# ChunLI-666/PointCloudProcessor

Hardware: AMD Instinct MI355X
Metric: Mpoints×frames/sec colorized (higher is better)
Workload: dtype f32/f64

## Files before the change

pointcloudprocessor_amd/csrc/pcp_colour.hip:

```cpp
#include <algorithm>
#include <cfloat>
#include <cstdlib>

#include "pcp_device.hpp"
#include "pcp_hsv.hpp"
#include "pcp_scan.hpp"

namespace pcp {

constexpr int kBlock = 256;
constexpr uint32_t kFltMaxBits = 0x7f7fffffu;

template <bool kCommon>
__device__ __forceinline__ DevCamera common_camera(const DevCamera &in) {
  DevCamera c = in;
  if constexpr (kCommon) {
    c.cull_mode = PCP_CULL_ZBUFFER;
    c.enable_zbuf = 1;
    c.pretest = 1;
    c.ds_fast = 1;
  }
  return c;
}
inline bool is_common_camera(const DevCamera &c) {
// ... 96 lines not shown
  double r = __builtin_amdgcn_rcp(b);
  r = fma(fma(-b, r, 1.0), r, r);
  r = fma(fma(-b, r, 1.0), r, r);
  return r;
}
__device__ __forceinline__ Interval iv_pad(Interval a) {
  const double e = 1e-12 * (fabs(a.lo) + fabs(a.hi)) + 1e-300;
  return {a.lo - e, a.hi + e};
}

__device__ __forceinline__ int tile_classify(const DevCamera &c, const DevFrame &fr, float4 sph) {
  const double cx = sph.x, cy = sph.y, cz = sph.z;
  const float *m = fr.w2c;
  const double X = (m[0] * cx + m[1] * cy) + (m[2] * cz + m[3]);
  const double Y = (m[4] * cx + m[5] * cy) + (m[6] * cz + m[7]);
  const double Z = (m[8] * cx + m[9] * cy) + (m[10] * cz + m[11]);
  const double mag = fr.norm_bound * (fabs(cx) + fabs(cy) + fabs(cz) + 3.0 * sph.w) + fabs(static_cast<double>(m[3])) +
                     fabs(static_cast<double>(m[7])) + fabs(static_cast<double>(m[11])) + 1e-3;
  const double rho = fr.norm_bound * static_cast<double>(sph.w) * (1.0 + 1e-6) + 1e-6 * mag;
  if (!(rho >= 0.0) || !isfinite(X + Y + Z + rho)) return 0;
  if (Z + rho <= 0.0) return 1;
  if (Z - rho <= 0.0) return 0;
  const Interval zi{Z - rho, Z + rho};
  if (!(zi.lo >= 1e-290)) return 0;
  const Interval iz{iv_rcp_pos(zi.hi) * (1.0 - 1e-13), iv_rcp_pos(zi.lo) * (1.0 + 1e-13)};
  const Interval xn = iv_pad(iv_mul_by_pos(Interval{X - rho, X + rho}, iz));
  const Interval yn = iv_pad(iv_mul_by_pos(Interval{Y - rho, Y + rho}, iz));
  const Interval x2 = iv_sqr(xn), y2 = iv_sqr(yn);
  const Interval r2 = iv_add(x2, y2);
  const Interval r4 = iv_mul_pos(r2, r2);
  const Interval r6 = iv_mul_pos(r2, r4);
  Interval rc = iv_add(iv_add(iv_scale(c.k1, r2), iv_scale(c.k2, r4)), iv_scale(c.k3, r6));
  rc.lo += 1.0;
  rc.hi += 1.0;
  const Interval t1 = iv_scale(2.0, iv_mul(xn, yn));
  const Interval t2 = iv_add(r2, iv_scale(2.0, x2));
  const Interval t3 = iv_add(r2, iv_scale(2.0, y2));
  const Interval xd = iv_pad(iv_add(iv_add(iv_mul(rc, xn), iv_scale(c.p1, t1)), iv_scale(c.p2, t2)));
  const Interval yd = iv_pad(iv_add(iv_add(iv_mul(rc, yn), iv_scale(c.p1, t3)), iv_scale(c.p2, t1)));
  Interval u = iv_pad(iv_scale(c.fx, xd)), v = iv_pad(iv_scale(c.fy, yd));
  u.lo += c.cx; u.hi += c.cx;
  v.lo += c.cy; v.hi += c.cy;
  if (!isfinite(u.lo + u.hi + v.lo + v.hi)) return 0;
  if (u.hi < static_cast<double>(c.u_lo) || u.lo > static_cast<double>(c.u_hi) ||
      v.hi < static_cast<double>(c.v_lo) || v.lo > static_cast<double>(c.v_hi))
    return 1;
  return (u.lo > static_cast<double>(c.u_lo) + 1.0 && u.hi < static_cast<double>(c.u_hi) - 1.0 &&
          v.lo > static_cast<double>(c.v_lo) + 1.0 && v.hi < static_cast<double>(c.v_hi) - 1.0)
             ? 2
             : 0;
}

constexpr int kTileGroup = 16;

__global__ __launch_bounds__(kBlock) void k_group_mask_flat(const float4 *__restrict__ spheres, int64_t groups, DevCamera cam,
                                                            const DevFrame *__restrict__ frames, int32_t n_frames,
                                                            int32_t w0, int32_t w1, int32_t words,
                                                            uint32_t *__restrict__ group_mask,
                                                            uint32_t *__restrict__ group_inside, int32_t cull_enabled,
                                                            int32_t *__restrict__ zeroed, int32_t n_zeroed,
                                                            unsigned long long *__restrict__ far_maps, int64_t far_cells) {
  const int64_t idx = static_cast<int64_t>(blockIdx.x) * kBlock + threadIdx.x;
  if (idx < n_zeroed) zeroed[idx] = 0;
  for (int64_t c = idx; c < far_cells; c += static_cast<int64_t>(gridDim.x) * kBlock) far_maps[c] = 0x7f7f7f7f7f7f7f7full;
  const int32_t nw = w1 - w0;
  const int64_t gw = idx >> 5;
  const int64_t group = gw / nw;
  const bool live = group < groups;
  const int32_t w = w0 + static_cast<int32_t>(gw - group * nw);
  const int32_t f = (w << 5) + static_cast<int32_t>(idx & 31);
  int cls = 1;
  if (live && f < n_frames) cls = cull_enabled ? tile_classify(cam, frames[f], spheres[group]) : 0;
  const unsigned long long m = __ballot(cls != 1), in = __ballot(cls == 2);
  if (live && (idx & 31) == 0) {
    group_mask[group * words + w] = static_cast<uint32_t>((threadIdx.x & 32) ? (m >> 32) : m);
    group_inside[group * words + w] = static_cast<uint32_t>((threadIdx.x & 32) ? (in >> 32) : in);
  }
}

__global__ __launch_bounds__(kBlock) void k_tile_mask_dense(const float4 *__restrict__ spheres, int64_t tiles,
                                                            DevCamera cam, const DevFrame *__restrict__ frames,
                                                            int32_t n_frames, int32_t w0, int32_t w1, int32_t words,
                                                            const uint32_t *__restrict__ group_mask,
                                                            const uint32_t *__restrict__ group_inside,
                                                            uint32_t *__restrict__ tile_mask,
                                                            uint32_t *__restrict__ inside_mask, int32_t cull_enabled) {
  const int lane = threadIdx.x & 63;
  const int32_t nw = w1 - w0;
  const int64_t gw = static_cast<int64_t>(blockIdx.x) * (kBlock / 64) + (threadIdx.x >> 6);
  const int64_t group = gw / nw;
  if (group >= (tiles + kTileGroup - 1) / kTileGroup) return;
  const int32_t w = w0 + static_cast<int32_t>(gw - group * nw);
  const int t = lane & 15, slot = lane >> 4;
  const int64_t tile = group * kTileGroup + t;
  const bool have = tile < tiles;
  uint32_t todo = __builtin_amdgcn_readfirstlane(group_mask[group * words + w]);
  const int32_t nb = n_frames - (w << 5);
  if (nb < 32) todo &= nb <= 0 ? 0u : ((1u << nb) - 1u);
  const uint32_t whole = __builtin_amdgcn_readfirstlane(group_inside[group * words + w]) & todo;
  todo &= ~whole;
  uint32_t word = whole, inside = whole;
  if (todo) {
    const float4 sph = spheres[have ? tile : tiles - 1];
    while (todo) {
      int32_t bit[4];
#pragma unroll
      for (int k = 0; k < 4; ++k) {
        bit[k] = todo ? __builtin_ctz(todo) : -1;
        todo &= todo - (todo ? 1u : 0u);
      }
      const int32_t b = slot == 0 ? bit[0] : slot == 1 ? bit[1] : slot == 2 ? bit[2] : bit[3];
      int cls = 1;
      if (b >= 0 && have) cls = cull_enabled ? tile_classify(cam, frames[(w << 5) + b], sph) : 0;
      const unsigned long long keep = __ballot(cls != 1), ins = __ballot(cls == 2);
#pragma unroll
      for (int k = 0; k < 4; ++k) {
        if (bit[k] >= 0) {
          word |= static_cast<uint32_t>((keep >> (k * 16 + t)) & 1ull) << bit[k];
          inside |= static_cast<uint32_t>((ins >> (k * 16 + t)) & 1ull) << bit[k];
        }
      }
    }
  }
  if (slot == 0 && have) {
    tile_mask[tile * words + w] = word;
    if (inside_mask) inside_mask[tile * words + w] = inside;
  }
}

constexpr int kWorkBins = 1024;
constexpr int kWorkPerBlock = 1024;
__global__ __launch_bounds__(kBlock) void k_tile_work_hist(const uint32_t *__restrict__ tile_mask, int64_t tiles, int32_t w0,
                                                          int32_t w1, int32_t words, int32_t *__restrict__ tile_work,
                                                          int32_t *__restrict__ hist) {
  __shared__ int32_t cnt[kWorkBins];
  for (int b = threadIdx.x; b < kWorkBins; b += kBlock) cnt[b] = 0;
  __syncthreads();
  const int64_t base = static_cast<int64_t>(blockIdx.x) * kWorkPerBlock;
  for (int q = 0; q < kWorkPerBlock / kBlock; ++q) {
    const int64_t t = base + q * kBlock + threadIdx.x;
    if (t < tiles) {
      int32_t visits = 0;
      for (int32_t w = w0; w < w1; ++w) visits += __builtin_popcount(tile_mask[t * words + w]);
      tile_work[t] = visits;
      atomicAdd(&cnt[min(visits, kWorkBins - 1)], 1);
    }
  }
  __syncthreads();
  for (int b = threadIdx.x; b < kWorkBins; b += kBlock)
    if (cnt[b]) atomicAdd(&hist[b], cnt[b]);
}
__device__ __forceinline__ int32_t block_exclusive_scan(int32_t v, int32_t *total);
__global__ __launch_bounds__(kBlock) void k_work_scatter(const int32_t *__restrict__ work, int64_t tiles,
                                                        const int32_t *__restrict__ hist, int32_t *__restrict__ cursor,
                                                        int32_t *__restrict__ order) {
  __shared__ int32_t cnt[kWorkBins];
  __shared__ int32_t first[kWorkBins];
  for (int b = threadIdx.x; b < kWorkBins; b += kBlock) cnt[b] = 0;
  {
    constexpr int kPer = kWorkBins / kBlock;
    int32_t h[kPer], mine = 0;
#pragma unroll
    for (int k = 0; k < kPer; ++k) {
      h[k] = hist[kWorkBins - 1 - (static_cast<int>(threadIdx.x) * kPer + k)];
      mine += h[k];
    }
    int32_t total = 0;
    int32_t run = block_exclusive_scan(mine, &total);
#pragma unroll
    for (int k = 0; k < kPer; ++k) {
      first[kWorkBins - 1 - (static_cast<int>(threadIdx.x) * kPer + k)] = run;
      run += h[k];
    }
  }
  __syncthreads();
  const int64_t base = static_cast<int64_t>(blockIdx.x) * kWorkPerBlock;
  int32_t bin[kWorkPerBlock / kBlock], rank[kWorkPerBlock / kBlock];
#pragma unroll
  for (int q = 0; q < kWorkPerBlock / kBlock; ++q) {
    const int64_t t = base + q * kBlock + threadIdx.x;
    bin[q] = t < tiles ? min(work[t], kWorkBins - 1) : -1;
    rank[q] = bin[q] >= 0 ? atomicAdd(&cnt[bin[q]], 1) : 0;
  }
  __syncthreads();
  for (int b = threadIdx.x; b < kWorkBins; b += kBlock)
    if (cnt[b]) cnt[b] = first[b] + atomicAdd(&cursor[b], cnt[b]);
  __syncthreads();
#pragma unroll
  for (int q = 0; q < kWorkPerBlock / kBlock; ++q)
    if (bin[q] >= 0) order[cnt[bin[q]] + rank[q]] = static_cast<int32_t>(base + q * kBlock + threadIdx.x);
}

constexpr uint32_t kXcdChunk = 16;
__device__ __forceinline__ uint32_t xcd_chunked_block() {
  constexpr uint32_t kXcd = 8, kSuper = kXcd * kXcdChunk;
  const uint32_t b = blockIdx.x;
  if (b >= (gridDim.x / kSuper) * kSuper) return b;
  const uint32_t x = b % kXcd, slot = b / kXcd;
  return ((slot / kXcdChunk) * kXcd + x) * kXcdChunk + slot % kXcdChunk;
}

constexpr unsigned long long kDepthEmpty = 0x7f7f7f7f7f7f7f7full;
__device__ __forceinline__ void depth_min(unsigned long long *__restrict__ map, int32_t cell, unsigned long long bits) {
  if (bits < map[cell]) atomicMin(map + cell, bits);
// ... 624 lines not shown
  if (need_frames && ctx->n_frames <= 0) return set_error(ctx, PCP_ERR_STATE, "%s: pcp_set_frames has not been called", who);
  hipError_t e = hipSetDevice(ctx->device);
  if (e != hipSuccess) return set_error(ctx, PCP_ERR_DEVICE, "%s: hipSetDevice failed: %s", who, hipGetErrorString(e));
  return PCP_OK;
}

static int check_frame(pcp_context *ctx, const char *who, int32_t frame) {
  if (frame < 0 || frame >= ctx->n_frames)
    return set_error(ctx, PCP_ERR_RANGE, "%s: keyframe %d out of range (0..%d)", who, frame, ctx->n_frames - 1);
  return PCP_OK;
}

static int fill_u32(pcp_context *ctx, uint32_t *p, int64_t n, uint32_t v) {
  if (n <= 0) return PCP_OK;
  LaunchTimer t(ctx, PCP_K_MISC);
  const uint32_t grid = static_cast<uint32_t>(std::min<int64_t>(div_up(n, kBlock), 8192));
  hipLaunchKernelGGL(k_fill_u32, dim3(grid), dim3(kBlock), 0, ctx->stream, p, n, v);
  PCP_HIP_TRY(ctx, hipGetLastError());
  return PCP_OK;
}

static int ensure_images(pcp_context *ctx) {
  const size_t px = static_cast<size_t>(ctx->dcam.img_w) * ctx->dcam.img_h;
  const size_t need = px * static_cast<size_t>(ctx->n_frames) + 4;
  if (ctx->images.count < need) {
    PCP_HIP_TRY(ctx, ctx->images.ensure(need));
    PCP_HIP_TRY(ctx, hipMemsetAsync(ctx->images.p, 0, need * 4, ctx->stream));
    ctx->image_set.assign(static_cast<size_t>(ctx->n_frames), 0);
    ctx->mask_set.assign(static_cast<size_t>(ctx->n_frames), 0);
  }
  return PCP_OK;
}

int wait_images(pcp_context *ctx, int32_t f0, int32_t f1) {
  ctx->texels_touched = true;
  if (ctx->image_pending.empty()) return PCP_OK;
  for (int lane = 0; lane < pcp_context::kUploadLanes; ++lane) {
    int32_t last = -1;
    for (int32_t f = std::max(f0, 0); f < f1 && f < static_cast<int32_t>(ctx->image_pending.size()); ++f) {
      const size_t sf = static_cast<size_t>(f);
      if (ctx->image_pending[sf] && ctx->image_lane[sf] == lane &&
          (last < 0 || ctx->image_seq[sf] > ctx->image_seq[static_cast<size_t>(last)]))
        last = f;
    }
    if (last < 0) continue;
    PCP_HIP_TRY(ctx, hipStreamWaitEvent(ctx->stream, ctx->image_event[static_cast<size_t>(last)], 0));
    const uint64_t seq = ctx->image_seq[static_cast<size_t>(last)];
    for (size_t f = 0; f < ctx->image_pending.size(); ++f)
      if (ctx->image_pending[f] && ctx->image_lane[f] == lane && ctx->image_seq[f] <= seq) ctx->image_pending[f] = 0;
  }
  return PCP_OK;
}

static int sort_tiles_by_work(pcp_context *ctx, int32_t w0, int32_t w1, int32_t *order) {
  const uint32_t sort_blocks = static_cast<uint32_t>(div_up(ctx->n_tiles, static_cast<int64_t>(kWorkPerBlock)));
  hipLaunchKernelGGL(k_tile_work_hist, dim3(sort_blocks), dim3(kBlock), 0, ctx->stream, ctx->tile_mask.p, ctx->n_tiles, w0, w1,
                     ctx->mask_words, ctx->tile_work.p, ctx->work_hist.p);
  hipLaunchKernelGGL(k_work_scatter, dim3(sort_blocks), dim3(kBlock), 0, ctx->stream, ctx->tile_work.p, ctx->n_tiles,
                     ctx->work_hist.p, ctx->work_hist.p + kWorkBins, order);
  PCP_HIP_TRY(ctx, hipGetLastError());
  return PCP_OK;
}

static int ensure_hull_bits(pcp_context *ctx) {
  const size_t words = static_cast<size_t>((ctx->n_frames + 31) / 32);
  const size_t need = words * static_cast<size_t>(ctx->n) + 4;
  if (ctx->hull_bits.count < need || ctx->hull_valid.size() != static_cast<size_t>(ctx->n_frames)) {
    PCP_HIP_TRY(ctx, ctx->hull_bits.ensure(need));
    ctx->hull_valid.assign(static_cast<size_t>(ctx->n_frames), 0);
  }
  return PCP_OK;
}

static int ensure_depth(pcp_context *ctx) {
  const size_t need = static_cast<size_t>(cells_of(ctx)) * ctx->n_frames + 4;
  if (ctx->depth.count < need) {
    PCP_HIP_TRY(ctx, ctx->depth.ensure(need));
    std::fill(ctx->depth_valid.begin(), ctx->depth_valid.end(), uint8_t(0));
  }
  const int32_t words = (ctx->n_frames + 31) / 32;
  const size_t need_mask = static_cast<size_t>(words) * static_cast<size_t>(std::max<int64_t>(ctx->n_tiles, 1)) + 4;
  if (ctx->tile_mask.count < need_mask || ctx->mask_words != words) {
    PCP_HIP_TRY(ctx, ctx->tile_mask.ensure(need_mask));
    PCP_HIP_TRY(ctx, ctx->tile_inside.ensure(need_mask));
    PCP_HIP_TRY(ctx, ctx->tile_work.ensure(static_cast<size_t>(std::max<int64_t>(ctx->n_tiles, 1)) + 4));
    PCP_HIP_TRY(ctx, ctx->tile_order.ensure(static_cast<size_t>(std::max<int64_t>(ctx->n_tiles, 1)) + 4));
    PCP_HIP_TRY(ctx, ctx->work_hist.ensure(2 * kWorkBins + 4));
    ctx->tile_order_live = false;
    ctx->mask_words = words;
    std::fill(ctx->depth_valid.begin(), ctx->depth_valid.end(), uint8_t(0));
  }
  return PCP_OK;
}

static int ensure_state(pcp_context *ctx) {
  const size_t sn = static_cast<size_t>(ctx->n);
  PCP_HIP_TRY(ctx, ctx->top_score.ensure(kTopM * sn + 4));
  PCP_HIP_TRY(ctx, ctx->top_rgb.ensure(kTopM * sn + 4));
  PCP_HIP_TRY(ctx, ctx->top_frame.ensure(kTopM * sn + 4));
  PCP_HIP_TRY(ctx, ctx->view_count.ensure(sn + 4));
  PCP_HIP_TRY(ctx, ctx->rgba2[0].ensure(sn + 4));
  PCP_HIP_TRY(ctx, ctx->rgba2[1].ensure(sn + 4));
  return PCP_OK;
}

int compact_flags(pcp_context *ctx, const uint8_t *flags, int64_t n, int32_t *out_index, int64_t capacity,
                  int64_t *count) {
  const int64_t tiles = std::max<int64_t>(1, div_up(n, kTile));
  PCP_HIP_TRY(ctx, ctx->s_tiles.ensure(static_cast<size_t>(tiles) + 4));
  PCP_HIP_TRY(ctx, ctx->s_counter.ensure(4));
  {
    LaunchTimer t(ctx, PCP_K_MISC);
    hipLaunchKernelGGL(k_tile_count, dim3(static_cast<uint32_t>(tiles)), dim3(kBlock), 0, ctx->stream, flags, n,
                       ctx->s_tiles.p);
    hipLaunchKernelGGL(k_scan_tiles, dim3(1), dim3(kScanTilesBlock), 0, ctx->stream, ctx->s_tiles.p, tiles, ctx->s_counter.p);
    if (out_index)
      hipLaunchKernelGGL(k_tile_scatter, dim3(static_cast<uint32_t>(tiles)), dim3(kBlock), 0, ctx->stream, flags, n,
                         ctx->s_tiles.p, out_index, capacity);
    PCP_HIP_TRY(ctx, hipGetLastError());
  }
  unsigned long long total = 0;
  unsigned long long *dst = ctx->readback ? static_cast<unsigned long long *>(ctx->readback) : &total;
  PCP_HIP_TRY(ctx, hipMemcpyAsync(dst, ctx->s_counter.p, sizeof(total), hipMemcpyDeviceToHost, ctx->stream));
  PCP_HIP_TRY(ctx, hipStreamSynchronize(ctx->stream));
  *count = static_cast<int64_t>(*dst);
  return PCP_OK;
}

static int single_frame_depth(pcp_context *ctx, int32_t frame) {
  const int64_t cells = cells_of(ctx);
  PCP_HIP_TRY(ctx, ctx->s_u32.ensure(static_cast<size_t>(cells) + 4));
  if (ctx->depth_from_batch) {
    if (!ctx->depth.p || static_cast<size_t>(frame) >= ctx->depth_valid.size() || !ctx->depth_valid[static_cast<size_t>(frame)])
      return set_error(ctx, PCP_ERR_STATE, "PCP_DEPTH_BATCHED: pcp_depth_pass has not covered keyframe %d", frame);
    PCP_HIP_TRY(ctx, hipMemcpyAsync(ctx->s_u32.p, ctx->depth.p + static_cast<int64_t>(frame) * cells,
                                    static_cast<size_t>(cells) * 4, hipMemcpyDeviceToDevice, ctx->stream));
    return PCP_OK;
  }
  if (ctx->n > 0 && ctx->dcam.enable_zbuf) {
    const size_t plane = plane_of(ctx);
// ... 465 lines not shown
    hipLaunchKernelGGL(k_gather_visible, dim3(blocks_for(take)), dim3(kBlock), 0, ctx->stream, ctx->xyz.p,
                       ctx->xyz.p + plane, ctx->xyz.p + 2 * plane, ctx->dcam, ctx->hframes[static_cast<size_t>(frame)],
                       ctx->s_cell.p, take, ctx->images.p + static_cast<int64_t>(frame) * px,
                       static_cast<int32_t>(ctx->image_set[static_cast<size_t>(frame)]),
                       static_cast<int32_t>(ctx->mask_set[static_cast<size_t>(frame)]),
                       reinterpret_cast<uint32_t *>(ctx->s_range.p), d_cam, d_world);
    PCP_HIP_TRY(ctx, hipGetLastError());
  }
  std::vector<uint32_t> rgbm;
  if (out_rgb || out_mask) {
    rgbm.resize(st);
    PCP_HIP_TRY(ctx, hipMemcpyAsync(rgbm.data(), ctx->s_range.p, st * 4, hipMemcpyDeviceToHost, ctx->stream));
  }
  if (out_index) PCP_HIP_TRY(ctx, hipMemcpyAsync(out_index, ctx->s_cell.p, st * 4, hipMemcpyDeviceToHost, ctx->stream));
  if (want_cam) PCP_HIP_TRY(ctx, hipMemcpyAsync(out_xyz_cam, d_cam, 3 * st * 4, hipMemcpyDeviceToHost, ctx->stream));
  if (want_world) PCP_HIP_TRY(ctx, hipMemcpyAsync(out_xyz_world, d_world, 3 * st * 4, hipMemcpyDeviceToHost, ctx->stream));
  PCP_HIP_TRY(ctx, hipStreamSynchronize(ctx->stream));
  for (size_t k = 0; k < rgbm.size(); ++k) {
    if (out_rgb) {
      out_rgb[3 * k + 0] = static_cast<uint8_t>(rgbm[k] & 0xffu);
      out_rgb[3 * k + 1] = static_cast<uint8_t>((rgbm[k] >> 8) & 0xffu);
      out_rgb[3 * k + 2] = static_cast<uint8_t>((rgbm[k] >> 16) & 0xffu);
    }
    if (out_mask) out_mask[k] = static_cast<uint16_t>(rgbm[k] >> 24);
  }
  return PCP_OK;
}

int pcp_depth_pass(pcp_context *ctx, int32_t frame_begin, int32_t frame_end) {
  int rc = check_ready(ctx, "pcp_depth_pass", true);
  if (rc != PCP_OK) return rc;
  if (frame_begin < 0 || frame_end > ctx->n_frames || frame_begin > frame_end)
    return set_error(ctx, PCP_ERR_RANGE, "pcp_depth_pass: keyframe range [%d,%d) outside 0..%d", frame_begin, frame_end,
                     ctx->n_frames);
  if (frame_begin == frame_end) return PCP_OK;
  if ((rc = ensure_depth(ctx)) != PCP_OK) return rc;
  const int64_t cells = cells_of(ctx);
  const int64_t map_cells = static_cast<int64_t>(frame_end - frame_begin) * cells;
  const bool z_maps = ctx->n > 0 && ctx->dcam.enable_zbuf;
  if (z_maps) {
    PCP_HIP_TRY(ctx, ctx->depth_sq.ensure(static_cast<size_t>(map_cells) + 4));
  } else if ((rc = fill_u32(ctx, ctx->depth.p + static_cast<int64_t>(frame_begin) * cells, map_cells, kFltMaxBits)) != PCP_OK) {
    return rc;
  }
  if (ctx->n > 0) {
    const size_t plane = plane_of(ctx);
    const int32_t w0 = frame_begin >> 5, w1 = ((frame_end - 1) >> 5) + 1;
    static const bool cull_tiles = [] {
      const char *e = std::getenv("PCP_DISABLE_TILE_CULL");
      return !(e && e[0] == '1');
    }();
    {
      LaunchTimer t(ctx, PCP_K_TILE_MASK);
      const int64_t groups = div_up(ctx->n_tiles, kTileGroup);
      const float4 *tile_sph = reinterpret_cast<const float4 *>(ctx->tile_sphere.p);
      const size_t gwords = static_cast<size_t>(groups) * ctx->mask_words;
      PCP_HIP_TRY(ctx, ctx->group_mask.ensure(2 * gwords + 8));
      uint32_t *group_inside = ctx->group_mask.p + gwords + 4;
      hipLaunchKernelGGL(k_group_mask_flat, dim3(std::max(blocks_for(groups * (w1 - w0) * 32), blocks_for(2 * kWorkBins))),
                         dim3(kBlock), 0, ctx->stream, tile_sph + ctx->n_tiles, groups, ctx->dcam, ctx->frames.p, ctx->n_frames,
                         w0, w1, ctx->mask_words, ctx->group_mask.p, group_inside, cull_tiles ? 1 : 0, ctx->work_hist.p,
                         2 * kWorkBins, z_maps ? reinterpret_cast<unsigned long long *>(ctx->depth_sq.p) : nullptr,
                         z_maps ? map_cells : int64_t(0));
      hipLaunchKernelGGL(k_tile_mask_dense, dim3(static_cast<uint32_t>(div_up(groups * (w1 - w0), kBlock / 64))), dim3(kBlock),
                         0, ctx->stream, tile_sph, ctx->n_tiles, ctx->dcam, ctx->frames.p, ctx->n_frames, w0, w1,
                         ctx->mask_words, ctx->group_mask.p, group_inside, ctx->tile_mask.p, ctx->tile_inside.p, cull_tiles ? 1 : 0);
      if ((rc = sort_tiles_by_work(ctx, w0, w1, ctx->tile_order.p)) != PCP_OK) return rc;
      ctx->tile_order_live = true;
    }
    if (ctx->cull.cull_mode == PCP_CULL_HPR) {
      int rch = ensure_hull_bits(ctx);
      if (rch != PCP_OK) return rch;
      if (!ctx->depth_from_batch) {
        int32_t clear_until = frame_begin;
        for (int32_t f = frame_begin; f < frame_end; ++f) {
          uint32_t *hull_plane = ctx->hull_bits.p + static_cast<size_t>(f >> 5) * static_cast<size_t>(ctx->n);
          if ((f & 31) == 0 && std::min(f + 32, ctx->n_frames) <= frame_end) {
            PCP_HIP_TRY(ctx, hipMemsetAsync(hull_plane, 0, static_cast<size_t>(ctx->n) * 4, ctx->stream));
            clear_until = std::min(f + 32, ctx->n_frames);
          }
          if (f >= clear_until) {
            LaunchTimer t(ctx, PCP_K_HPR);
            hipLaunchKernelGGL(k_hull_clear, dim3(blocks_for(ctx->n)), dim3(kBlock), 0, ctx->stream, hull_plane, ctx->n, 1u << (f & 31));
          }
        }
        PCP_HIP_TRY(ctx, hipGetLastError());
        const char *le = std::getenv("PCP_HPR_LANES");
        const int32_t lanes = le && le[0] >= '1' && le[0] <= '8' ? le[0] - '0' : 4;
        if ((rc = hpr_run_range(ctx, frame_begin, frame_end, lanes, ctx->tile_mask.p)) != PCP_OK) return rc;
        for (int32_t f = frame_begin; f < frame_end; ++f) ctx->hull_valid[static_cast<size_t>(f)] = 1;
      }
    }
    {
      LaunchTimer t(ctx, PCP_K_DEPTH);
      hipLaunchKernelGGL(is_common_camera(ctx->dcam) ? k_depth_pass<true> : k_depth_pass<false>,
                         dim3(static_cast<uint32_t>(ctx->n_tiles)), dim3(64), 0, ctx->stream, ctx->sxyz.p,
                         ctx->sxyz.p + plane, ctx->sxyz.p + 2 * plane, ctx->n, ctx->dcam, ctx->frames.p, frame_begin,
                         frame_end, ctx->depth_sq.p, cells, frame_begin, ctx->tile_mask.p, ctx->tile_inside.p,
                         ctx->mask_words, ctx->tile_order.p);
      if (z_maps)
        hipLaunchKernelGGL(k_depth_finish, dim3(static_cast<uint32_t>(std::min<int64_t>(div_up(map_cells, kBlock), 4096))),
                           dim3(kBlock), 0, ctx->stream, ctx->depth_sq.p, map_cells,
                           ctx->depth.p + static_cast<int64_t>(frame_begin) * cells);
      PCP_HIP_TRY(ctx, hipGetLastError());
    }
  }
  for (int32_t f = frame_begin; f < frame_end; ++f) ctx->depth_valid[static_cast<size_t>(f)] = 1;
  return PCP_OK;
}

int pcp_depth_maps_device(pcp_context *ctx, void **device_ptr, int64_t *n_floats) {
  int rc = check_ready(ctx, "pcp_depth_maps_device", true);
  if (rc != PCP_OK) return rc;
  if (ctx->cull.cull_mode == PCP_CULL_HPR)
    return set_error(ctx, PCP_ERR_STATE, "pcp_depth_maps_device: PCP_CULL_HPR has no depth maps to merge across point shards "
                     "(the hull needs the whole map on one GPU)");
  if ((rc = ensure_depth(ctx)) != PCP_OK) return rc;
  if (device_ptr) *device_ptr = ctx->depth.p;
  if (n_floats) *n_floats = cells_of(ctx) * ctx->n_frames;
  return PCP_OK;
// ... 427 lines not shown
```

pointcloudprocessor_amd/csrc/pcp_context.hip:

```cpp
#include <algorithm>
#include <cfloat>
#include <cmath>
#include <cstdlib>
#include <new>
#include <vector>

#include "pcp_internal.hpp"
#include "pcp_scan.hpp"

namespace pcp {

static thread_local std::string g_error;

int set_error(const pcp_context *ctx, int code, const char *fmt, ...) {
  char buf[1024];
  va_list ap;
  va_start(ap, fmt);
  vsnprintf(buf, sizeof(buf), fmt, ap);
  va_end(ap);
  if (ctx)
    ctx->error = buf;
  else
    g_error = buf;
  return code;
// ... 428 lines not shown

static int store_cloud(pcp_context *ctx, const float *x, const float *y, const float *z, int64_t n,
                       const void *aos = nullptr, int64_t stride = 0) {
  PCP_HIP_TRY(ctx, hipSetDevice(ctx->device));
  const size_t sn = static_cast<size_t>(n);
  const size_t plane = (sn + 3) & ~size_t(3);
  PCP_HIP_TRY(ctx, ctx->xyz.ensure(3 * plane + 4));
  PCP_HIP_TRY(ctx, ctx->sxyz.ensure(3 * plane + 4));
  PCP_HIP_TRY(ctx, ctx->perm.ensure(sn + 4));
  ctx->n = n;
  ctx->nonfinite_points = 0;
  ctx->sor_distances_live = false;
  ctx->sor_partial_slab = ctx->sor_partial_slabs = -1;
  ctx->n_tiles = 0;
  ctx->tile_order_live = false;
  ctx->have_intensity = false;
  ctx->nid_chunks = 0;
  ctx->colour_state_live = false;
  ctx->colour_result_live = false;
  ctx->labels_live = false;
  match_table_release(ctx);
  ctx->mls_count = 0;
  ctx->vgd_next = ctx->css_next = -1;
  ctx->css_ball = 0.0;
  std::fill(ctx->depth_valid.begin(), ctx->depth_valid.end(), uint8_t(0));
  ctx->hull_valid.clear();
  for (int a = 0; a < 3; ++a) ctx->host_min[a] = ctx->host_max[a] = 0.0f;
  if (n == 0) return PCP_OK;
  hipStream_t st = ctx->stream;
  float *dx = ctx->xyz.p, *dy = ctx->xyz.p + plane, *dz = ctx->xyz.p + 2 * plane;
  PCP_HIP_TRY(ctx, hipMemsetAsync(ctx->sxyz.p, 0, (3 * plane + 4) * 4, st));
  DevBuf<uint32_t> raw;
  if (aos) {
    PCP_HIP_TRY(ctx, raw.ensure(static_cast<size_t>(n) * static_cast<size_t>(stride) / 4 + 4));
    PCP_HIP_TRY(ctx, hipMemcpyAsync(raw.p, aos, static_cast<size_t>(n) * static_cast<size_t>(stride), hipMemcpyHostToDevice, st));
    hipLaunchKernelGGL(k_up_deinterleave, dim3(up_blocks(n)), dim3(kUpBlock), 0, st, raw.p, stride / 4, n, dx, dy, dz);
  } else {
    PCP_HIP_TRY(ctx, hipMemcpyAsync(dx, x, sn * 4, hipMemcpyHostToDevice, st));
    PCP_HIP_TRY(ctx, hipMemcpyAsync(dy, y, sn * 4, hipMemcpyHostToDevice, st));
    PCP_HIP_TRY(ctx, hipMemcpyAsync(dz, z, sn * 4, hipMemcpyHostToDevice, st));
  }
  float mn[3], mx[3];
  unsigned long long nonfinite = 0;
  PCP_HIP_TRY(ctx, ctx->inv_perm.ensure(plane + 4));
  if (int rc = spatial_order(ctx, dx, dy, dz, n, ctx->perm.p, ctx->sxyz.p, ctx->sxyz.p + plane, ctx->sxyz.p + 2 * plane,
                             ctx->inv_perm.p, mn, mx, &nonfinite))
    return rc;
  raw.release();
  ctx->nonfinite_points = static_cast<int64_t>(nonfinite);
  for (int a = 0; a < 3; ++a) {
    ctx->host_min[a] = mn[a];
    ctx->host_max[a] = mx[a];
  }
  const int64_t tiles = (n + 63) / 64, groups = (tiles + 15) / 16;
  PCP_HIP_TRY(ctx, ctx->tile_sphere.ensure(static_cast<size_t>(tiles + groups) * 4 + 4));
  float4 *sph = reinterpret_cast<float4 *>(ctx->tile_sphere.p);
  hipLaunchKernelGGL(k_up_spheres<64>, dim3(static_cast<uint32_t>((tiles + 3) / 4)), dim3(kUpBlock), 0, st, ctx->sxyz.p,
                     ctx->sxyz.p + plane, ctx->sxyz.p + 2 * plane, n, sph, tiles);
  hipLaunchKernelGGL(k_up_spheres<1024>, dim3(static_cast<uint32_t>(groups)), dim3(kUpBlock), 0, st, ctx->sxyz.p,
                     ctx->sxyz.p + plane, ctx->sxyz.p + 2 * plane, n, sph + tiles, groups);
  PCP_HIP_TRY(ctx, hipGetLastError());
  ctx->n_tiles = tiles;
  PCP_HIP_TRY(ctx, hipStreamSynchronize(st));
  return PCP_OK;
}

}

using namespace pcp;

extern "C" {

int pcp_abi_version(void) { return PCP_ABI_VERSION; }

int pcp_create(int32_t device, pcp_context **out) {
  if (!out) {
    set_global_error("pcp_create: out is NULL");
    return PCP_ERR_INVALID;
  }
  *out = nullptr;
  int count = 0;
  hipError_t e = hipGetDeviceCount(&count);
  if (e != hipSuccess || count <= 0) {
    set_global_error("pcp_create: no HIP device available (%s); libpcp_hip has no CPU fallback",
                     e == hipSuccess ? "device count 0" : hipGetErrorString(e));
    return PCP_ERR_DEVICE;
  }
  if (device < 0 || device >= count) {
    set_global_error("pcp_create: device %d out of range (0..%d)", device, count - 1);
    return PCP_ERR_INVALID;
  }
  e = hipSetDevice(device);
  if (e == hipSuccess) {
    hipFuncAttributes a;
    const hipError_t pl[] = {hipFuncGetAttributes(&a, reinterpret_cast<const void *>(&k_up_bbox)), preload_colour(), preload_mls(),
                             preload_nid(), preload_hpr(), preload_colour_smooth(), preload_match(),
                             preload_jpeg()};
    for (hipError_t x : pl)
      if (x != hipSuccess && e == hipSuccess) e = x;
  }
  if (e != hipSuccess) {
    set_global_error("pcp_create: hipSetDevice(%d) / loading the gfx950 code objects failed: %s", device, hipGetErrorString(e));
    return PCP_ERR_DEVICE;
  }
  pcp_context *ctx = new (std::nothrow) pcp_context();
  if (!ctx) {
    set_global_error("pcp_create: out of host memory");
    return PCP_ERR_NOMEM;
  }
  ctx->device = device;
  e = hipStreamCreateWithFlags(&ctx->own_stream, hipStreamNonBlocking);
  if (e != hipSuccess) {
    set_global_error("pcp_create: hipStreamCreate failed: %s", hipGetErrorString(e));
// ... 7 lines not shown
    if (e == hipSuccess) e = hipStreamCreateWithPriority(&ctx->copy_stream, hipStreamNonBlocking, prio_greatest);
  }
  for (int k = 0; k < 2 && e == hipSuccess; ++k) {
    e = hipEventCreateWithFlags(&ctx->result_ready[k], hipEventDisableTiming);
    if (e == hipSuccess) e = hipEventCreateWithFlags(&ctx->copy_done[k], hipEventDisableTiming);
  }
  if (e != hipSuccess) {
    set_global_error("pcp_create: copy stream / events: %s", hipGetErrorString(e));
    pcp_destroy(ctx);
    return PCP_ERR_DEVICE;
  }
  if (hipHostMalloc(&ctx->readback, pcp_context::kReadbackBytes, hipHostMallocDefault) != hipSuccess) {
    ctx->readback = nullptr;
    (void)hipGetLastError();
  }
  pcp_default_camera(&ctx->camera);
  pcp_default_cull_params(&ctx->cull);
  *out = ctx;
  return PCP_OK;
}

void pcp_destroy(pcp_context *ctx) {
  if (!ctx) return;
  (void)hipSetDevice(ctx->device);
  (void)hipStreamSynchronize(ctx->stream);
  if (ctx->copy_stream) (void)hipStreamSynchronize(ctx->copy_stream);
  for (hipStream_t us : ctx->upload_stream)
    if (us) {
      (void)hipStreamSynchronize(us);
      (void)hipStreamDestroy(us);
    }
  for (auto e : ctx->image_event)
    if (e) (void)hipEventDestroy(e);
  if (ctx->texels_idle) (void)hipEventDestroy(ctx->texels_idle);
  for (auto &b : ctx->upload_stage) b.release();
  for (auto &b : ctx->jpeg_planes) b.release();
  drain_timing(ctx);
  for (auto e : ctx->event_pool) (void)hipEventDestroy(e);
  ctx->xyz.release();
  ctx->sxyz.release();
  ctx->perm.release();
  ctx->inv_perm.release();
  ctx->frames.release();
  ctx->images.release();
  ctx->hsv_tables.release();
  ctx->depth.release();
  ctx->depth_sq.release();
  ctx->tile_sphere.release();
  ctx->tile_mask.release();
  ctx->tile_inside.release();
  ctx->tile_work.release();
  ctx->tile_order.release();
  ctx->work_hist.release();
  ctx->group_mask.release();
  ctx->top_score.release();
  ctx->top_rgb.release();
  ctx->top_frame.release();
  ctx->view_count.release();
  ctx->rgba2[0].release();
  ctx->rgba2[1].release();
  ctx->labels.release();
  match_table_release(ctx);
  ctx->match_moved.release();
  for (int k = 0; k < 2; ++k) {
    if (ctx->result_ready[k]) (void)hipEventDestroy(ctx->result_ready[k]);
    if (ctx->copy_done[k]) (void)hipEventDestroy(ctx->copy_done[k]);
  }
  if (ctx->copy_stream) (void)hipStreamDestroy(ctx->copy_stream);
  ctx->s_cell.release();
  ctx->s_pixel.release();
  ctx->s_range.release();
  ctx->s_cam.release();
  ctx->s_keep.release();
  ctx->s_u32.release();
  ctx->s_counter.release();
  ctx->s_tiles.release();
  ctx->g_cell.release();
  ctx->g_rank.release();
  ctx->g_start.release();
  ctx->g_occ.release();
  ctx->g_occ_rank.release();
  ctx->g_order.release();
  ctx->g_xyz.release();
  ctx->m_tmp.release();
  ctx->s_dist.release();
  ctx->css_dist.release();
  ctx->s_kth.release();
  ctx->css_words.release();
  ctx->m_state.release();
  ctx->slp_table.release();
  ctx->c_perm.release();
  ctx->m_flag.release();
  ctx->intensity.release();
  for (auto &lane : ctx->hpr_lane) lane.release();
  if (ctx->hpr_fork) (void)hipEventDestroy(ctx->hpr_fork);
  for (auto &e : ctx->hpr_join)
    if (e) (void)hipEventDestroy(e);
  ctx->hull_bits.release();
  ctx->nid_pts.release();
  ctx->nid_chunk_kf.release();
  ctx->nid_hist.release();
  ctx->m_sums.release();
  ctx->c_index.release();
  ctx->c_xyz.release();
  ctx->c_mark.release();
  ctx->c_where.release();
  ctx->c_xyz2.release();
// ... 299 lines not shown
```

pointcloudprocessor_amd/csrc/pcp_internal.hpp:

```cpp
#pragma once

#include <hip/hip_runtime.h>

#include <cstdarg>
#include <cstdint>
#include <chrono>
#include <cstdio>
#include <cstring>
#include <string>
#include <vector>

#include "pcp_hip.h"

namespace pcp {

struct DevCamera {
  double fx, fy, cx, cy;
  double k1, k2, p1, p2, k3;
  double slack;
  float ds_f;
  double img_wd, img_hd;
  float cull_wf, cull_hf;
  float ds_rcp;
  int32_t ds_fast;
// ... 107 lines not shown
}

struct pcp_context {
  int32_t device = 0;
  hipStream_t own_stream = nullptr;
  hipStream_t stream = nullptr;
  void *readback = nullptr;
  static constexpr size_t kReadbackBytes = 65536;
  mutable std::string error;

  bool have_camera = false;
  pcp_camera camera{};
  pcp_cull_params cull{};
  pcp::DevCamera dcam{};

  int64_t n = 0;
  int64_t nonfinite_points = 0;
  pcp::DevBuf<float> xyz;
  pcp::DevBuf<float> sxyz;
  pcp::DevBuf<int32_t> perm;
  pcp::DevBuf<int32_t> inv_perm;
  std::vector<float> host_min = {0, 0, 0}, host_max = {0, 0, 0};

  int32_t n_frames = 0;
  std::vector<pcp_pose> poses;
  std::vector<pcp::DevFrame> hframes;
  pcp::DevBuf<pcp::DevFrame> frames;
  pcp::DevBuf<uint32_t> images;
  std::vector<uint8_t> image_set, mask_set;
  static constexpr int kUploadLanes = 2;
  hipStream_t upload_stream[kUploadLanes] = {nullptr, nullptr};
  pcp::DevBuf<uint8_t> upload_stage[kUploadLanes];
  pcp::DevBuf<uint8_t> jpeg_planes[kUploadLanes];
  std::vector<hipEvent_t> image_event;
  std::vector<uint8_t> image_pending;
  std::vector<uint8_t> image_lane;
  std::vector<uint64_t> image_seq;
  bool lane_must_wait[kUploadLanes] = {false, false};
  uint64_t upload_seq = 0;
  uint64_t upload_turn = 0;
  hipEvent_t texels_idle = nullptr;
  bool texels_touched = false;
  bool adjust_images = false;
  float saturation_scale = 1.0f, brightness_scale = 1.0f;
  pcp::DevBuf<int32_t> hsv_tables;

  pcp::DevBuf<uint32_t> depth;
  pcp::DevBuf<unsigned long long> depth_sq;
  std::vector<uint8_t> depth_valid;
  bool depth_from_batch = false;

  int64_t n_tiles = 0;
  pcp::DevBuf<float> tile_sphere;
  pcp::DevBuf<uint32_t> tile_mask, group_mask;
  pcp::DevBuf<uint32_t> tile_inside;
  int32_t mask_words = 0;
  pcp::DevBuf<int32_t> tile_work, tile_order, work_hist;
  bool tile_order_live = false;

  pcp::DevBuf<float> top_score;
  pcp::DevBuf<uint32_t> top_rgb;
  pcp::DevBuf<int32_t> top_frame;
  pcp::DevBuf<int32_t> view_count;
  pcp::DevBuf<uint32_t> rgba2[2];
  int32_t rgba_cur = 0;
  hipStream_t copy_stream = nullptr;
  hipEvent_t result_ready[2] = {nullptr, nullptr}, copy_done[2] = {nullptr, nullptr};
  bool copy_pending[2] = {false, false};
  bool colour_state_live = false;
  bool colour_result_live = false;
  bool label_fusion = false;
  bool labels_live = false;
  pcp::DevBuf<uint32_t> labels;

  bool match_live = false;
  double match_e = 0.0, match_rc = 0.0;
  float match_e2 = 0.0f;
  int64_t match_a = 0;
  int64_t match_entries = 0;
  pcp::DevBuf<uint8_t> match_in_a;
  pcp::DevBuf<int32_t> match_list;
  pcp::DevBuf<int64_t> match_off;
  pcp::DevBuf<int32_t> match_cols;
  pcp::DevBuf<unsigned long long> match_moved;

  pcp::DevBuf<int32_t> s_cell, s_pixel;
  pcp::DevBuf<float> s_range, s_cam;
  pcp::DevBuf<uint8_t> s_keep;
  pcp::DevBuf<uint32_t> s_u32;
  pcp::DevBuf<unsigned long long> s_counter;
  pcp::DevBuf<int32_t> s_tiles;

  static constexpr int kHprMaxLanes = 8;
  pcp::HprLane hpr_lane[kHprMaxLanes];
  int32_t hpr_last_lane = 0;
  hipEvent_t hpr_fork = nullptr, hpr_join[kHprMaxLanes] = {};
  pcp::DevBuf<uint32_t> hull_bits;
  std::vector<uint8_t> hull_valid;
  int64_t hpr_stats[10] = {0, 0, 0, 0, 0, 0, 0, 0, 0, 0};
  bool hpr_stats_pending = false;

  pcp::DevBuf<int32_t> g_cell, g_rank, g_start, g_order;
  pcp::DevBuf<unsigned long long> g_occ;
  pcp::DevBuf<int32_t> g_occ_rank;
  pcp::DevBuf<float> g_xyz;
  pcp::DevBuf<float> m_tmp;
  pcp::DevBuf<float> s_dist;
  pcp::DevBuf<double> m_state;
  double slp_radius = 0.05, slp_step = 0.01;
  pcp::DevBuf<float> slp_table;
// ... 145 lines not shown
```

Before: 1.871 million.

## Fuse hierarchical tile culling, work histogram into one three-level mask kernel

Replaces the separate group-mask, dense tile-mask and work-histogram kernels with one kernel per block of tile groups. It adds a third, coarser level of bounding spheres (16 groups each) and culls hierarchically with shared-memory append lists. The histogram is computed in the same kernel, and its counters are double-buffered so each launch zeroes the next set. This removes two launches and a global re-read of the tile masks, and skips per-tile tests for frames rejected at the upper or group level. The cost is heavier shared-memory use and serialized loops over frame chunks within each block.

New measurement: 1.901 million, median of 6. Within noise of the previous version (+1.6%).

```diff
diff --git a/pointcloudprocessor_amd/csrc/pcp_colour.hip b/pointcloudprocessor_amd/csrc/pcp_colour.hip
--- a/pointcloudprocessor_amd/csrc/pcp_colour.hip
+++ b/pointcloudprocessor_amd/csrc/pcp_colour.hip
@@ -172,104 +172,127 @@
 }
 
 constexpr int kTileGroup = 16;
-
-__global__ __launch_bounds__(kBlock) void k_group_mask_flat(const float4 *__restrict__ spheres, int64_t groups, DevCamera cam,
-                                                            const DevFrame *__restrict__ frames, int32_t n_frames,
-                                                            int32_t w0, int32_t w1, int32_t words,
-                                                            uint32_t *__restrict__ group_mask,
-                                                            uint32_t *__restrict__ group_inside, int32_t cull_enabled,
-                                                            int32_t *__restrict__ zeroed, int32_t n_zeroed,
-                                                            unsigned long long *__restrict__ far_maps, int64_t far_cells) {
-  const int64_t idx = static_cast<int64_t>(blockIdx.x) * kBlock + threadIdx.x;
-  if (idx < n_zeroed) zeroed[idx] = 0;
-  for (int64_t c = idx; c < far_cells; c += static_cast<int64_t>(gridDim.x) * kBlock) far_maps[c] = 0x7f7f7f7f7f7f7f7full;
-  const int32_t nw = w1 - w0;
-  const int64_t gw = idx >> 5;
-  const int64_t group = gw / nw;
-  const bool live = group < groups;
-  const int32_t w = w0 + static_cast<int32_t>(gw - group * nw);
-  const int32_t f = (w << 5) + static_cast<int32_t>(idx & 31);
-  int cls = 1;
-  if (live && f < n_frames) cls = cull_enabled ? tile_classify(cam, frames[f], spheres[group]) : 0;
-  const unsigned long long m = __ballot(cls != 1), in = __ballot(cls == 2);
-  if (live && (idx & 31) == 0) {
-    group_mask[group * words + w] = static_cast<uint32_t>((threadIdx.x & 32) ? (m >> 32) : m);
-    group_inside[group * words + w] = static_cast<uint32_t>((threadIdx.x & 32) ? (in >> 32) : in);
-  }
-}
-
-__global__ __launch_bounds__(kBlock) void k_tile_mask_dense(const float4 *__restrict__ spheres, int64_t tiles,
-                                                            DevCamera cam, const DevFrame *__restrict__ frames,
-                                                            int32_t n_frames, int32_t w0, int32_t w1, int32_t words,
-                                                            const uint32_t *__restrict__ group_mask,
-                                                            const uint32_t *__restrict__ group_inside,
-                                                            uint32_t *__restrict__ tile_mask,
-                                                            uint32_t *__restrict__ inside_mask, int32_t cull_enabled) {
+constexpr int kUpperGroups = 16;
+#ifndef PCP_MASK_GROUPS
+#define PCP_MASK_GROUPS 4
+#endif
+constexpr int kMaskGroups = PCP_MASK_GROUPS;
+constexpr int kMaskTiles = kMaskGroups * kTileGroup;
+constexpr int kMaskChunkWords = kBlock / 32;
+static_assert(kUpperGroups % kMaskGroups == 0 && kMaskTiles <= kBlock, "a workgroup lies within one upper group");
+#ifndef PCP_MASK_UPPER
+#define PCP_MASK_UPPER 1
+#endif
+constexpr bool kMaskUpper = PCP_MASK_UPPER != 0;
+constexpr int kWorkBins = 1024;
+
+__device__ __forceinline__ void wave_append(bool take, uint16_t v, uint16_t *list, int32_t *count) {
+  const unsigned long long b = __ballot(take);
+  if (!b) return;
   const int lane = threadIdx.x & 63;
-  const int32_t nw = w1 - w0;
-  const int64_t gw = static_cast<int64_t>(blockIdx.x) * (kBlock / 64) + (threadIdx.x >> 6);
-  const int64_t group = gw / nw;
-  if (group >= (tiles + kTileGroup - 1) / kTileGroup) return;
-  const int32_t w = w0 + static_cast<int32_t>(gw - group * nw);
-  const int t = lane & 15, slot = lane >> 4;
-  const int64_t tile = group * kTileGroup + t;
-  const bool have = tile < tiles;
-  uint32_t todo = __builtin_amdgcn_readfirstlane(group_mask[group * words + w]);
-  const int32_t nb = n_frames - (w << 5);
-  if (nb < 32) todo &= nb <= 0 ? 0u : ((1u << nb) - 1u);
-  const uint32_t whole = __builtin_amdgcn_readfirstlane(group_inside[group * words + w]) & todo;
-  todo &= ~whole;
-  uint32_t word = whole, inside = whole;
-  if (todo) {
-    const float4 sph = spheres[have ? tile : tiles - 1];
-    while (todo) {
-      int32_t bit[4];
-#pragma unroll
-      for (int k = 0; k < 4; ++k) {
-        bit[k] = todo ? __builtin_ctz(todo) : -1;
-        todo &= todo - (todo ? 1u : 0u);
+  int32_t base = 0;
+  if (lane == 0) base = atomicAdd(count, static_cast<int32_t>(__popcll(b)));
+  base = __shfl(base, 0, 64);
+  if (take) list[base + static_cast<int32_t>(__popcll(b & ((1ull << lane) - 1ull)))] = v;
+}
+
+__global__ __launch_bounds__(kBlock) void k_mask_stage(const float4 *__restrict__ spheres, int64_t tiles, DevCamera cam,
+                                                       const DevFrame *__restrict__ frames, int32_t n_frames, int32_t w0,
+                                                       int32_t w1, int32_t words, uint32_t *__restrict__ tile_mask,
+                                                       uint32_t *__restrict__ inside_mask, int32_t *__restrict__ tile_work,
+                                                       int32_t *__restrict__ hist, int32_t cull_enabled,
+                                                       int32_t *__restrict__ zeroed, int32_t n_zeroed,
+                                                       unsigned long long *__restrict__ far_maps, int64_t far_cells) {
+  __shared__ uint16_t l0[kBlock];
+  __shared__ uint16_t l1[kMaskGroups * kBlock];
+  __shared__ uint32_t up_in[kMaskChunkWords];
+  __shared__ uint32_t g_in[kMaskGroups][kMaskChunkWords];
+  __shared__ uint32_t t_keep[kMaskTiles][kMaskChunkWords], t_in[kMaskTiles][kMaskChunkWords];
+  __shared__ int32_t t_work[kMaskTiles];
+  __shared__ int32_t cnt[kWorkBins];
+  __shared__ int32_t n0, n1;
+  const int tid = threadIdx.x;
+  const int64_t idx = static_cast<int64_t>(blockIdx.x) * kBlock + tid, stride = static_cast<int64_t>(gridDim.x) * kBlock;
+  for (int64_t c = idx; c < n_zeroed; c += stride) zeroed[c] = 0;
+  for (int64_t c = idx; c < far_cells; c += stride) far_maps[c] = 0x7f7f7f7f7f7f7f7full;
+  const int64_t groups = (tiles + kTileGroup - 1) / kTileGroup;
+  const int64_t group0 = static_cast<int64_t>(blockIdx.x) * kMaskGroups, tile0 = group0 * kTileGroup;
+  const float4 *group_sph = spheres + tiles, *upper_sph = group_sph + groups;
+  for (int b = tid; b < kWorkBins; b += kBlock) cnt[b] = 0;
+  if (tid < kMaskTiles) t_work[tid] = 0;
+  __syncthreads();
+  for (int32_t wc = w0; wc < w1; wc += kMaskChunkWords) {
+    const int32_t nwc = min(kMaskChunkWords, w1 - wc), f_base = wc << 5;
+    if (cull_enabled) {
+      for (int i = tid; i < kMaskTiles * kMaskChunkWords; i += kBlock) (&t_keep[0][0])[i] = (&t_in[0][0])[i] = 0u;
+      if (tid < kMaskGroups * kMaskChunkWords) (&g_in[0][0])[tid] = 0u;
+      if (tid == 0) n0 = n1 = 0;
+      __syncthreads();
+      {
+        const bool valid = tid < nwc * 32 && f_base + tid < n_frames;
+        int cls = 1;
+        if (valid) cls = kMaskUpper ? tile_classify(cam, frames[f_base + tid], upper_sph[group0 / kUpperGroups]) : 0;
+        const unsigned long long in = __ballot(cls == 2);
+        if ((tid & 63) == 0) {
+          up_in[(tid >> 6) * 2] = static_cast<uint32_t>(in);
+          up_in[(tid >> 6) * 2 + 1] = static_cast<uint32_t>(in >> 32);
+        }
+        wave_append(cls == 0, static_cast<uint16_t>(tid), l0, &n0);
       }
-      const int32_t b = slot == 0 ? bit[0] : slot == 1 ? bit[1] : slot == 2 ? bit[2] : bit[3];
-      int cls = 1;
-      if (b >= 0 && have) cls = cull_enabled ? tile_classify(cam, frames[(w << 5) + b], sph) : 0;
-      const unsigned long long keep = __ballot(cls != 1), ins = __ballot(cls == 2);
-#pragma unroll
-      for (int k = 0; k < 4; ++k) {
-        if (bit[k] >= 0) {
-          word |= static_cast<uint32_t>((keep >> (k * 16 + t)) & 1ull) << bit[k];
-          inside |= static_cast<uint32_t>((ins >> (k * 16 + t)) & 1ull) << bit[k];
-        }
+      __syncthreads();
+      const int32_t m1 = n0 * kMaskGroups;
+      for (int32_t i0 = 0; i0 < m1; i0 += kBlock) {
+        const int32_t i = i0 + tid;
+        const int32_t kf = i < m1 ? l0[i / kMaskGroups] : 0, g = i % kMaskGroups;
+        int cls = 1;
+        if (i < m1 && group0 + g < groups) cls = tile_classify(cam, frames[f_base + kf], group_sph[group0 + g]);
+        if (cls == 2) atomicOr(&g_in[g][kf >> 5], 1u << (kf & 31));
+        wave_append(cls == 0, static_cast<uint16_t>((g << 8) | kf), l1, &n1);
       }
-    }
-  }
-  if (slot == 0 && have) {
-    tile_mask[tile * words + w] = word;
-    if (inside_mask) inside_mask[tile * words + w] = inside;
-  }
-}
-
-constexpr int kWorkBins = 1024;
+      __syncthreads();
+      const int32_t m2 = n1 * kTileGroup;
+      for (int32_t i0 = 0; i0 < m2; i0 += kBlock) {
+        const int32_t i = i0 + tid;
+        const int32_t e = i < m2 ? l1[i >> 4] : 0;
+        const int32_t kf = e & 255, tl = (e >> 8) * kTileGroup + (i & 15);
+        int cls = 1;
+        if (i < m2 && tile0 + tl < tiles) cls = tile_classify(cam, frames[f_base + kf], spheres[tile0 + tl]);
+        if (cls != 1) atomicOr(&t_keep[tl][kf >> 5], 1u << (kf & 31));
+        if (cls == 2) atomicOr(&t_in[tl][kf >> 5], 1u << (kf & 31));
+      }
+      __syncthreads();
+    }
+    for (int32_t i = tid; i < kMaskTiles * nwc; i += kBlock) {
+      const int32_t tl = i / nwc, j = i - tl * nwc;
+      if (tile0 + tl >= tiles) continue;
+      uint32_t word, inside = 0u;
+      if (cull_enabled) {
+        inside = up_in[j] | g_in[tl / kTileGroup][j];
+        word = t_keep[tl][j] | inside;
+        inside |= t_in[tl][j];
+      } else {
+        const int32_t nb = n_frames - ((wc + j) << 5);
+        word = nb >= 32 ? 0xffffffffu : nb <= 0 ? 0u : ((1u << nb) - 1u);
+      }
+      tile_mask[(tile0 + tl) * words + wc + j] = word;
+      inside_mask[(tile0 + tl) * words + wc + j] = inside;
+      atomicAdd(&t_work[tl], static_cast<int32_t>(__builtin_popcount(word)));
+    }
+    __syncthreads();
+  }
+  int32_t bin = -1;
+  bool first = false;
+  if (tid < kMaskTiles && tile0 + tid < tiles) {
+    const int32_t visits = t_work[tid];
+    tile_work[tile0 + tid] = visits;
+    bin = min(visits, kWorkBins - 1);
+    first = atomicAdd(&cnt[bin], 1) == 0;
+  }
+  __syncthreads();
+  if (first) atomicAdd(&hist[bin], cnt[bin]);
+}
+
 constexpr int kWorkPerBlock = 1024;
-__global__ __launch_bounds__(kBlock) void k_tile_work_hist(const uint32_t *__restrict__ tile_mask, int64_t tiles, int32_t w0,
-                                                          int32_t w1, int32_t words, int32_t *__restrict__ tile_work,
-                                                          int32_t *__restrict__ hist) {
-  __shared__ int32_t cnt[kWorkBins];
-  for (int b = threadIdx.x; b < kWorkBins; b += kBlock) cnt[b] = 0;
-  __syncthreads();
-  const int64_t base = static_cast<int64_t>(blockIdx.x) * kWorkPerBlock;
-  for (int q = 0; q < kWorkPerBlock / kBlock; ++q) {
-    const int64_t t = base + q * kBlock + threadIdx.x;
-    if (t < tiles) {
-      int32_t visits = 0;
-      for (int32_t w = w0; w < w1; ++w) visits += __builtin_popcount(tile_mask[t * words + w]);
-      tile_work[t] = visits;
-      atomicAdd(&cnt[min(visits, kWorkBins - 1)], 1);
-    }
-  }
-  __syncthreads();
-  for (int b = threadIdx.x; b < kWorkBins; b += kBlock)
-    if (cnt[b]) atomicAdd(&hist[b], cnt[b]);
-}
 __device__ __forceinline__ int32_t block_exclusive_scan(int32_t v, int32_t *total);
 __global__ __launch_bounds__(kBlock) void k_work_scatter(const int32_t *__restrict__ work, int64_t tiles,
                                                         const int32_t *__restrict__ hist, int32_t *__restrict__ cursor,
@@ -1000,16 +1023,6 @@
   return PCP_OK;
 }
 
-static int sort_tiles_by_work(pcp_context *ctx, int32_t w0, int32_t w1, int32_t *order) {
-  const uint32_t sort_blocks = static_cast<uint32_t>(div_up(ctx->n_tiles, static_cast<int64_t>(kWorkPerBlock)));
-  hipLaunchKernelGGL(k_tile_work_hist, dim3(sort_blocks), dim3(kBlock), 0, ctx->stream, ctx->tile_mask.p, ctx->n_tiles, w0, w1,
-                     ctx->mask_words, ctx->tile_work.p, ctx->work_hist.p);
-  hipLaunchKernelGGL(k_work_scatter, dim3(sort_blocks), dim3(kBlock), 0, ctx->stream, ctx->tile_work.p, ctx->n_tiles,
-                     ctx->work_hist.p, ctx->work_hist.p + kWorkBins, order);
-  PCP_HIP_TRY(ctx, hipGetLastError());
-  return PCP_OK;
-}
-
 static int ensure_hull_bits(pcp_context *ctx) {
   const size_t words = static_cast<size_t>((ctx->n_frames + 31) / 32);
   const size_t need = words * static_cast<size_t>(ctx->n) + 4;
@@ -1033,7 +1046,11 @@
     PCP_HIP_TRY(ctx, ctx->tile_inside.ensure(need_mask));
     PCP_HIP_TRY(ctx, ctx->tile_work.ensure(static_cast<size_t>(std::max<int64_t>(ctx->n_tiles, 1)) + 4));
     PCP_HIP_TRY(ctx, ctx->tile_order.ensure(static_cast<size_t>(std::max<int64_t>(ctx->n_tiles, 1)) + 4));
-    PCP_HIP_TRY(ctx, ctx->work_hist.ensure(2 * kWorkBins + 4));
+    if (ctx->work_hist.count < 4 * kWorkBins + 4) {
+      PCP_HIP_TRY(ctx, ctx->work_hist.ensure(4 * kWorkBins + 4));
+      PCP_HIP_TRY(ctx, hipMemsetAsync(ctx->work_hist.p, 0, 4 * kWorkBins * sizeof(int32_t), ctx->stream));
+      ctx->work_hist_set = 0;
+    }
     ctx->tile_order_live = false;
     ctx->mask_words = words;
     std::fill(ctx->depth_valid.begin(), ctx->depth_valid.end(), uint8_t(0));
@@ -1605,20 +1622,20 @@
     }();
     {
       LaunchTimer t(ctx, PCP_K_TILE_MASK);
+      const float4 *tile_sph = reinterpret_cast<const float4 *>(ctx->tile_sphere.p);
       const int64_t groups = div_up(ctx->n_tiles, kTileGroup);
-      const float4 *tile_sph = reinterpret_cast<const float4 *>(ctx->tile_sphere.p);
-      const size_t gwords = static_cast<size_t>(groups) * ctx->mask_words;
-      PCP_HIP_TRY(ctx, ctx->group_mask.ensure(2 * gwords + 8));
-      uint32_t *group_inside = ctx->group_mask.p + gwords + 4;
-      hipLaunchKernelGGL(k_group_mask_flat, dim3(std::max(blocks_for(groups * (w1 - w0) * 32), blocks_for(2 * kWorkBins))),
-                         dim3(kBlock), 0, ctx->stream, tile_sph + ctx->n_tiles, groups, ctx->dcam, ctx->frames.p, ctx->n_frames,
-                         w0, w1, ctx->mask_words, ctx->group_mask.p, group_inside, cull_tiles ? 1 : 0, ctx->work_hist.p,
+      int32_t *counters = ctx->work_hist.p + ctx->work_hist_set * 2 * kWorkBins;
+      int32_t *next_counters = ctx->work_hist.p + (ctx->work_hist_set ^ 1) * 2 * kWorkBins;
+      ctx->work_hist_set ^= 1;
+      hipLaunchKernelGGL(k_mask_stage, dim3(static_cast<uint32_t>(div_up(groups, kMaskGroups))), dim3(kBlock), 0, ctx->stream,
+                         tile_sph, ctx->n_tiles, ctx->dcam, ctx->frames.p, ctx->n_frames, w0, w1, ctx->mask_words,
+                         ctx->tile_mask.p, ctx->tile_inside.p, ctx->tile_work.p, counters, cull_tiles ? 1 : 0, next_counters,
                          2 * kWorkBins, z_maps ? reinterpret_cast<unsigned long long *>(ctx->depth_sq.p) : nullptr,
                          z_maps ? map_cells : int64_t(0));
-      hipLaunchKernelGGL(k_tile_mask_dense, dim3(static_cast<uint32_t>(div_up(groups * (w1 - w0), kBlock / 64))), dim3(kBlock),
-                         0, ctx->stream, tile_sph, ctx->n_tiles, ctx->dcam, ctx->frames.p, ctx->n_frames, w0, w1,
-                         ctx->mask_words, ctx->group_mask.p, group_inside, ctx->tile_mask.p, ctx->tile_inside.p, cull_tiles ? 1 : 0);
-      if ((rc = sort_tiles_by_work(ctx, w0, w1, ctx->tile_order.p)) != PCP_OK) return rc;
+      hipLaunchKernelGGL(k_work_scatter, dim3(static_cast<uint32_t>(div_up(ctx->n_tiles, static_cast<int64_t>(kWorkPerBlock)))),
+                         dim3(kBlock), 0, ctx->stream, ctx->tile_work.p, ctx->n_tiles, counters, counters + kWorkBins,
+                         ctx->tile_order.p);
+      PCP_HIP_TRY(ctx, hipGetLastError());
       ctx->tile_order_live = true;
     }
     if (ctx->cull.cull_mode == PCP_CULL_HPR) {
diff --git a/pointcloudprocessor_amd/csrc/pcp_context.hip b/pointcloudprocessor_amd/csrc/pcp_context.hip
--- a/pointcloudprocessor_amd/csrc/pcp_context.hip
+++ b/pointcloudprocessor_amd/csrc/pcp_context.hip
@@ -504,13 +504,15 @@
     ctx->host_min[a] = mn[a];
     ctx->host_max[a] = mx[a];
   }
-  const int64_t tiles = (n + 63) / 64, groups = (tiles + 15) / 16;
-  PCP_HIP_TRY(ctx, ctx->tile_sphere.ensure(static_cast<size_t>(tiles + groups) * 4 + 4));
+  const int64_t tiles = (n + 63) / 64, groups = (tiles + 15) / 16, uppers = (groups + 15) / 16;
+  PCP_HIP_TRY(ctx, ctx->tile_sphere.ensure(static_cast<size_t>(tiles + groups + uppers) * 4 + 4));
   float4 *sph = reinterpret_cast<float4 *>(ctx->tile_sphere.p);
   hipLaunchKernelGGL(k_up_spheres<64>, dim3(static_cast<uint32_t>((tiles + 3) / 4)), dim3(kUpBlock), 0, st, ctx->sxyz.p,
                      ctx->sxyz.p + plane, ctx->sxyz.p + 2 * plane, n, sph, tiles);
   hipLaunchKernelGGL(k_up_spheres<1024>, dim3(static_cast<uint32_t>(groups)), dim3(kUpBlock), 0, st, ctx->sxyz.p,
                      ctx->sxyz.p + plane, ctx->sxyz.p + 2 * plane, n, sph + tiles, groups);
+  hipLaunchKernelGGL(k_up_spheres<16384>, dim3(static_cast<uint32_t>(uppers)), dim3(kUpBlock), 0, st, ctx->sxyz.p,
+                     ctx->sxyz.p + plane, ctx->sxyz.p + 2 * plane, n, sph + tiles + groups, uppers);
   PCP_HIP_TRY(ctx, hipGetLastError());
   ctx->n_tiles = tiles;
   PCP_HIP_TRY(ctx, hipStreamSynchronize(st));
@@ -624,7 +626,6 @@
   ctx->tile_work.release();
   ctx->tile_order.release();
   ctx->work_hist.release();
-  ctx->group_mask.release();
   ctx->top_score.release();
   ctx->top_rgb.release();
   ctx->top_frame.release();
diff --git a/pointcloudprocessor_amd/csrc/pcp_internal.hpp b/pointcloudprocessor_amd/csrc/pcp_internal.hpp
--- a/pointcloudprocessor_amd/csrc/pcp_internal.hpp
+++ b/pointcloudprocessor_amd/csrc/pcp_internal.hpp
@@ -183,10 +183,11 @@
 
   int64_t n_tiles = 0;
   pcp::DevBuf<float> tile_sphere;
-  pcp::DevBuf<uint32_t> tile_mask, group_mask;
+  pcp::DevBuf<uint32_t> tile_mask;
   pcp::DevBuf<uint32_t> tile_inside;
   int32_t mask_words = 0;
   pcp::DevBuf<int32_t> tile_work, tile_order, work_hist;
+  int32_t work_hist_set = 0;
   bool tile_order_live = false;
 
   pcp::DevBuf<float> top_score;
```
